# olehskip/resnet.c

Measured on AMD Instinct MI355X. Metric: images/sec ResNet-50 224x224 fp32 batch=256, higher is better.
Workload: dtype f32; 1 GPU; resnet50 fp32 forward, batch 256 per GPU, 224x224 (BASELINE.json configs[2]); global_batch=256, batch_per_gpu=256, mode=fused conv+bn+relu(+add) epilogues, streams_per_gpu=2, streams_configured=library default, front_parts=1, parallelism=batch split over 1 GPU(s), weights replicated, no collective

## Files before the change

### include/rn_hip.h

```cpp
#ifndef RN_HIP_H
#define RN_HIP_H

#include <stddef.h>
#include <stdint.h>

#ifdef __cplusplus
extern "C" {
#endif

#if defined(__GNUC__)
#define RN_API __attribute__((visibility("default")))
#else
#define RN_API
#endif

typedef struct rn_ctx rn_ctx;
typedef struct rn_model rn_model;
typedef struct rn_event rn_event;

enum {
    RN_OK = 0,
    RN_ERR_INVALID = 1,
    RN_ERR_HIP = 2,
    RN_ERR_IO = 3,
// ... 16 lines not shown
RN_API int rn_ctx_get_layout(const rn_ctx *ctx);
RN_API int rn_ctx_set_sync_each_op(rn_ctx *ctx, int on);
RN_API int rn_ctx_set_deferred(rn_ctx *ctx, int on);
RN_API int rn_ctx_get_deferred(const rn_ctx *ctx);
RN_API int rn_flush(rn_ctx *ctx);
RN_API int rn_observe(rn_ctx *ctx, const void *dev_ptr);
RN_API int rn_ctx_deferred_stats(const rn_ctx *ctx, uint64_t *pending_ops, uint64_t *nhwc_buffers,
                                 uint64_t *fused_launches, uint64_t *literal_launches,
                                 uint64_t *transposes);
RN_API int rn_ctx_set_weight_cache(rn_ctx *ctx, int on);
RN_API uint64_t rn_ctx_launch_count(const rn_ctx *ctx);
RN_API int rn_conv_tile_candidates(void);
RN_API int rn_ctx_set_conv_tile(rn_ctx *ctx, int candidate);
RN_API int rn_ctx_set_split_k(rn_ctx *ctx, int max_splits);
RN_API int rn_ctx_set_stem_items(rn_ctx *ctx, int items);
RN_API int rn_ctx_set_xcd_groups(rn_ctx *ctx, int groups);
RN_API int rn_ctx_set_nchw_taps(rn_ctx *ctx, int mode);
RN_API int rn_ctx_set_tap_skip(rn_ctx *ctx, int mode);
RN_API int rn_ctx_tap_skip_stats(const rn_ctx *ctx, uint64_t *launches, uint64_t *k_tiles_skipped);
RN_API int rn_conv_tap_skip_plan(int dtype, uint64_t B, uint64_t in_channels, uint64_t out_channels, uint64_t H,
                                 uint64_t W, uint64_t kernel_size, uint64_t stride, uint64_t padding,
                                 uint64_t dilation, int tile, uint64_t *m_tiles, uint64_t *k_tiles,
                                 uint64_t *k_tiles_skipped, int *rule);
RN_API int rn_ctx_set_debug_stamps(rn_ctx *ctx, void *dev_buffer);
RN_API void *rn_ctx_stream(rn_ctx *ctx);
RN_API int rn_ctx_device(const rn_ctx *ctx);
RN_API int rn_sync(rn_ctx *ctx);
RN_API const char *rn_last_error(const rn_ctx *ctx);
RN_API const char *rn_status_string(int status);
RN_API int rn_device_count(int *count);
RN_API int rn_device_locality(int device, char *pci_bus_id, uint64_t pci_cap, int *numa_node,
                              char *cpulist, uint64_t cpulist_cap);
RN_API const char *rn_version(void);

RN_API int rn_malloc(rn_ctx *ctx, void **dev_ptr, uint64_t bytes);
RN_API int rn_free(rn_ctx *ctx, void *dev_ptr);
RN_API int rn_memcpy_h2d(rn_ctx *ctx, void *dev_dst, const void *host_src, uint64_t bytes);
RN_API int rn_memcpy_d2h(rn_ctx *ctx, void *host_dst, const void *dev_src, uint64_t bytes);
RN_API int rn_memcpy_d2d(rn_ctx *ctx, void *dev_dst, const void *dev_src, uint64_t bytes);
RN_API int rn_memset(rn_ctx *ctx, void *dev_ptr, int byte_value, uint64_t bytes);
RN_API int rn_load_f32_file(rn_ctx *ctx, const char *path, float **dev_ptr, uint64_t *numel);
RN_API int rn_save_f32_file(rn_ctx *ctx, const char *path, const float *dev_ptr, uint64_t numel);

RN_API int rn_event_create(rn_ctx *ctx, rn_event **out);
RN_API int rn_event_destroy(rn_event *ev);
RN_API int rn_event_record(rn_ctx *ctx, rn_event *ev);
// ... 359 lines not shown
```

### resnet.c_amd/_lib.py

```python
from __future__ import annotations

import ctypes
import os
from ctypes import POINTER, c_char_p, c_double, c_float, c_int, c_uint64, c_void_p

_HERE = os.path.dirname(os.path.abspath(__file__))
LIB_PATH = os.environ.get("RN_HIP_LIB") or os.path.join(_HERE, "librn_hip.so")

RN_OK = 0
RN_ERR_INVALID, RN_ERR_HIP, RN_ERR_IO, RN_ERR_NOMEM, RN_ERR_UNSUPPORTED = 1, 2, 3, 4, 5
RN_LAYOUT_NCHW, RN_LAYOUT_NHWC = 0, 1
RN_FWD_REFERENCE_OPS, RN_FWD_FUSED = 0, 1
RN_DTYPE_F32, RN_DTYPE_BF16 = 0, 1
RN_CONV_MAX_DILATION = 1024

u64 = c_uint64
fptr = c_void_p


class ConvSecond(ctypes.Structure):
    _fields_ = [("inp", c_void_p), ("in_channels", c_uint64), ("H", c_uint64), ("W", c_uint64),
                ("stride", c_uint64)]


# ... 20 lines not shown


SIGNATURES = {
    "rn_ctx_create": (c_int, [POINTER(c_void_p), c_int, c_void_p]),
    "rn_ctx_destroy": (c_int, [c_void_p]),
    "rn_ctx_set_layout": (c_int, [c_void_p, c_int]),
    "rn_ctx_get_layout": (c_int, [c_void_p]),
    "rn_ctx_set_sync_each_op": (c_int, [c_void_p, c_int]),
    "rn_ctx_set_deferred": (c_int, [c_void_p, c_int]),
    "rn_ctx_get_deferred": (c_int, [c_void_p]),
    "rn_flush": (c_int, [c_void_p]),
    "rn_observe": (c_int, [c_void_p, c_void_p]),
    "rn_ctx_deferred_stats": (c_int, [c_void_p] + [POINTER(u64)] * 5),
    "rn_ctx_set_weight_cache": (c_int, [c_void_p, c_int]),
    "rn_ctx_launch_count": (u64, [c_void_p]),
    "rn_conv_tile_candidates": (c_int, []),
    "rn_ctx_set_conv_tile": (c_int, [c_void_p, c_int]),
    "rn_ctx_set_split_k": (c_int, [c_void_p, c_int]),
    "rn_ctx_set_stem_items": (c_int, [c_void_p, c_int]),
    "rn_ctx_set_xcd_groups": (c_int, [c_void_p, c_int]),
    "rn_ctx_set_nchw_taps": (c_int, [c_void_p, c_int]),
    "rn_ctx_set_tap_skip": (c_int, [c_void_p, c_int]),
    "rn_ctx_tap_skip_stats": (c_int, [c_void_p, POINTER(u64), POINTER(u64)]),
    "rn_conv_tap_skip_plan": (c_int, [c_int] + [u64] * 9 + [c_int] + [POINTER(u64)] * 3 + [POINTER(c_int)]),
    "rn_ctx_set_debug_stamps": (c_int, [c_void_p, c_void_p]),
    "rn_ctx_stream": (c_void_p, [c_void_p]),
    "rn_ctx_device": (c_int, [c_void_p]),
    "rn_sync": (c_int, [c_void_p]),
    "rn_last_error": (c_char_p, [c_void_p]),
    "rn_status_string": (c_char_p, [c_int]),
    "rn_device_count": (c_int, [POINTER(c_int)]),
    "rn_device_locality": (c_int, [c_int, c_char_p, u64, POINTER(c_int), c_char_p, u64]),
    "rn_version": (c_char_p, []),
    "rn_malloc": (c_int, [c_void_p, POINTER(c_void_p), u64]),
    "rn_free": (c_int, [c_void_p, c_void_p]),
    "rn_memcpy_h2d": (c_int, [c_void_p, c_void_p, c_void_p, u64]),
    "rn_memcpy_d2h": (c_int, [c_void_p, c_void_p, c_void_p, u64]),
    "rn_memcpy_d2d": (c_int, [c_void_p, c_void_p, c_void_p, u64]),
    "rn_memset": (c_int, [c_void_p, c_void_p, c_int, u64]),
    "rn_load_f32_file": (c_int, [c_void_p, c_char_p, POINTER(c_void_p), POINTER(u64)]),
    "rn_save_f32_file": (c_int, [c_void_p, c_char_p, c_void_p, u64]),
    "rn_event_create": (c_int, [c_void_p, POINTER(c_void_p)]),
    "rn_event_destroy": (c_int, [c_void_p]),
    "rn_event_record": (c_int, [c_void_p, c_void_p]),
    "rn_event_elapsed_ms": (c_int, [c_void_p, c_void_p, POINTER(c_float)]),
    "rn_conv_output_size": (u64, [u64, u64, u64, u64]),
# ... 230 lines not shown
```

### resnet.c_amd/csrc/rn_conv.hip

```cpp
#include <type_traits>

#include "rn_conv_params.h"
#include "rn_private.h"

bool rn_conv_is_c4(uint64_t Cin, uint64_t k);

using namespace rn_gemm;

namespace {

constexpr int ROW_FLOATS = 32;

constexpr int tile_blocks_per_cu(int BM, int BN) { return BM * BN <= 64 * 64 ? 4 : BM * BN <= 64 * 128 ? 3 : 2; }

template <typename T, typename TO, int BM, int BN, bool DUAL = false, bool XK = false, bool CHUNK = false,
          bool DIL = false, bool PM = false>
__global__ __launch_bounds__(256, tile_blocks_per_cu(BM, BN)) void conv_gemm_kernel(const GemmParams p)
{
    constexpr int CH = Elem<T>::CH, ES = (int)sizeof(T);
    constexpr int AP = BM / 32;
    constexpr int BP = BN / 32;
    constexpr int MI = BM / 64;
    constexpr int NI = BN / 64;
    constexpr int STAGE = (BM + BN) * ROW_FLOATS;
    __shared__ __attribute__((aligned(16))) float lds[2 * STAGE];

    __builtin_amdgcn_s_setprio(3);
    stamp(p.stamps, 0);
    const unsigned total_tiles = CHUNK ? p.full_tiles : p.total_tiles;
    auto logical_origin = [&](unsigned logical, int &m0_, int &n0_) {
        n0_ = (int)(logical % (unsigned)p.tiles_n) * BN;
        m0_ = (int)(logical / (unsigned)p.tiles_n) * BM;
    };
    auto tile_origin = [&](unsigned v, int &m0_, int &n0_) {
        unsigned pos = xcd_deal(total_tiles, v);
        if (p.xg > 0) {
            const unsigned xg = (unsigned)p.xg, per_group = p.xrows * xg;
            if (pos < p.xrows * (unsigned)p.tiles_n) {
                const unsigned grp = pos / per_group, rem = pos - grp * per_group;
                const unsigned mp = rem / xg, nn = rem - mp * xg;
                pos = mp * (unsigned)p.tiles_n + grp * xg + nn;
            }
        }
        logical_origin(pos, m0_, n0_);
    };
    auto work_item = [&](unsigned v, int &m0_, int &n0_, int &kb_, int &ke_, int &s_) {
        if constexpr (CHUNK) {
            if (v >= p.full_tiles) {
                const unsigned qq = v - p.full_tiles, chunk = qq / p.tail_tiles;
                logical_origin(p.full_tiles + (qq - chunk * p.tail_tiles), m0_, n0_);
                kb_ = (int)chunk * p.chunk_L;
                ke_ = min(kb_ + p.chunk_L, p.nk);
                s_ = (int)chunk;
            } else {
                tile_origin(v, m0_, n0_);
                kb_ = 0;
                ke_ = p.nk;
                s_ = -1;
// ... 929 lines not shown
        auto cost = [&](int g) {
            const double nt = (double)tn / g, mp = R / nt < 1 ? 1 : R / nt;
            const bool stays = taps ? nt * w_slab + mp * a_slab <= 3.8 * MB : nt * w_slab <= 2.5 * MB;
            const double generations = panels / (8.0 / g) / mp;
            const double again = stays ? 1.0 : 3.0 * (generations < 1 ? 1 : generations);
            if (taps && !stays && g > 1) return 1e300;
            return (g > 1 ? 1.3 : 1.0) * g * A + 8.0 * (Wb / g) * again;
        };
        groups = 1;
        double best = cost(1);
        for (int g = 2; g <= 8; g *= 2) {
            if (tn % (unsigned)g) break;
            const double c = cost(g);
            if (c < 0.8 * best) best = c, groups = g;
        }
    }
    if (groups > 8) groups = 8;
    while (groups > 1 && tn % (unsigned)groups) groups /= 2;
    if (groups <= 1) return;
    p.xg = (int)(tn / (unsigned)groups);
    p.xrows = remap_tiles / tn;
}

template <typename T, typename TO, int BM, int BN, bool DUAL, bool XK, bool CHUNK, bool DIL, bool PM>
void launch_one(rn_ctx *ctx, const GemmParams &p, bool persistent, int *occupancy)
{
    unsigned grid = p.grid_items;
    if (persistent) {
        if (*occupancy == 0) {
            int nb = 0;
            if (hipOccupancyMaxActiveBlocksPerMultiprocessor(
                    &nb, conv_gemm_kernel<T, TO, BM, BN, DUAL, XK, CHUNK, DIL, PM>, 256, 0) != hipSuccess ||
                nb < 1)
                nb = 1;
            *occupancy = nb;
        }
        const unsigned slots = 256u * (unsigned)*occupancy;
        if (grid > slots) grid = slots;
    }
    conv_gemm_kernel<T, TO, BM, BN, DUAL, XK, CHUNK, DIL, PM><<<dim3(grid), dim3(256), 0, ctx->stream>>>(p);
}

struct KernelRow {
    int dt_in, dt_out, BM, BN;
    bool dual, xk, chunk, dil, pm;
    void (*launch)(rn_ctx *, const GemmParams &, bool persistent, int *occupancy);
// ... 43 lines not shown
        r.launch(ctx, p, c.persistent, &ctx->occupancy[&r - kKernels]);
        return rn_after_launch(ctx, d.what);
    }
    if (d.second) return rn_set_error(ctx, RN_ERR_UNSUPPORTED, "%s: fused pair needs equal in/out dtype", d.what);
    return rn_set_error(ctx, RN_ERR_UNSUPPORTED, "%s: dtype combination %d -> %d", d.what, d.dt_in, d.dt_out);
}

int launch_gemm(rn_ctx *ctx, const Contraction &d)
{
    GemmParams p = describe(ctx, d);
    const Choice c = choose(ctx, d, p);
    if (c.family == Choice::STRIP) {
        rn_conv_strip_launch(ctx, p);
        return rn_after_launch(ctx, d.what);
    }
    if (c.family == Choice::FOUR_WAVE && ctx->tap_skip != 1) {
        const TapSkipPlan t = plan_tap_skip(d, p, c.BM, c.BN, ctx->split_k > 1);
        if (t.eligible && (ctx->tap_skip == 2 || t.rule)) {
            Choice cp = c;
            cp.pm = true;
            RN_REQUIRE(ctx, split_pixel_major(p, d, c.BM, c.BN), "too many tiles");
            if (c.chunked) p.chunk_L = 2 * (int)rn_ceil_div((uint64_t)p.nk, 16);
            else p.chunk_L = p.nk;
            choose_tile_order(ctx, p, p.full_tiles, c.BM, c.BN);
            RN_TRY(dispatch(ctx, d, cp, p, false));
            ctx->tap_skip_launches += 1, ctx->tap_skip_k_tiles += t.k_skipped;
            return RN_OK;
        }
    }
    RN_REQUIRE(ctx, split_whole_tiles(p, c.BM, c.BN), "too many tiles");
    if (c.family == Choice::WIDE) {
        rn_conv_wide_launch(ctx, p, c.which, d.second != nullptr);
        return rn_after_launch(ctx, d.what);
    }
    FinishParams fin{};
    RN_TRY(split_k_loop(ctx, d, p, &fin));
    const bool k_split = fin.splits > 0;
    if (!k_split) {
        if (c.chunked) RN_TRY(split_chunked_tail(ctx, d, c.BM, p, &fin));
        choose_tile_order(ctx, p, p.full_tiles, c.BM, c.BN);
    }
    RN_TRY(dispatch(ctx, d, c, p, k_split));
    if (fin.splits == 0) return RN_OK;
    const unsigned fgrid = rn_stream_grid(fin.slice / 4, 256);
    if (d.dt_out == RN_DTYPE_BF16)
        splitk_finish_kernel<bf16_t><<<fgrid, 256, 0, ctx->stream>>>(fin);
    else
// ... 236 lines not shown
    if ((dtype != RN_DTYPE_F32 && dtype != RN_DTYPE_BF16) || tile < 0 || tile > 8 || B == 0 || in_channels == 0 ||
        out_channels == 0 || kernel_size == 0 || kernel_size > 15 || stride == 0 || dilation == 0)
        return -1;
    const uint64_t h_out = rn_conv_output_size_dilated(H, kernel_size, stride, padding, dilation);
    const uint64_t w_out = rn_conv_output_size_dilated(W, kernel_size, stride, padding, dilation);
    if (h_out == 0 || w_out == 0) return -1;
    if (dtype != RN_DTYPE_F32 || in_channels % 32 != 0 ||
        !gemm_eligible(nullptr, nullptr, nullptr, in_channels, kernel_size, B * H * W * in_channels,
                       out_channels * kernel_size * kernel_size * in_channels, B * h_out * w_out * out_channels))
        return 0;
    Contraction d{};
    d.dt_in = d.dt_out = dtype;
    d.k = kernel_size, d.stride = stride, d.pad = padding, d.dil = kernel_size == 1 ? 1 : dilation;
    d.h_out = h_out, d.w_out = w_out, d.B = B, d.Cin = in_channels, d.Cout = out_channels, d.H = H, d.W = W;
    rn_ctx none{};
    const GemmParams p = describe(&none, d);
    const Choice c = choose_four_wave(tile, d, p);
    const TapSkipPlan t = plan_tap_skip(d, p, c.BM, c.BN, false);
    if (!t.eligible) return 0;
    if (m_tiles) *m_tiles = t.m_tiles;
    if (k_tiles) *k_tiles = t.k_tiles;
    if (k_tiles_skipped) *k_tiles_skipped = t.k_skipped;
    if (rule) *rule = t.rule ? 1 : 0;
    return 1;
}

int rn_conv2d_nhwc_forward(rn_ctx *ctx, const float *inp, float *out, const float *packed_weight,
                           uint64_t kernel_size, uint64_t stride, uint64_t padding, uint64_t h_out,
                           uint64_t w_out, uint64_t B, uint64_t in_channels, uint64_t out_channels,
                           uint64_t H, uint64_t W, const rn_epilogue *epilogue)
{
    return nhwc_forward(ctx, inp, out, packed_weight, kernel_size, stride, padding, 1, h_out, w_out, B, in_channels,
                        out_channels, H, W, epilogue);
}

int rn_conv2d_forward(rn_ctx *ctx, const float *inp, float *out, const float *weight,
                      uint64_t kernel_size, uint64_t stride, uint64_t padding, uint64_t h_out,
                      uint64_t w_out, uint64_t B, uint64_t in_channels, uint64_t out_channels,
                      uint64_t H, uint64_t W)
{
    return conv2d_forward(ctx, inp, out, weight, kernel_size, stride, padding, 1, h_out, w_out, B, in_channels,
                          out_channels, H, W);
}

int rn_conv2d_nhwc_forward_dt(rn_ctx *ctx, int dtype, int out_dtype, const void *inp, void *out,
                              const void *packed_weight, uint64_t kernel_size, uint64_t stride,
// ... 174 lines not shown
```

### resnet.c_amd/csrc/rn_conv_params.h

```cpp
#ifndef RN_CONV_PARAMS_H
#define RN_CONV_PARAMS_H

#include "rn_internal.h"

namespace rn_gemm {

typedef float f32x16 __attribute__((ext_vector_type(16)));
typedef unsigned int u32x4 __attribute__((ext_vector_type(4)));

struct GemmParams {
    const void *in;
    const void *w;
    void *out;
    const float *scale;
    const float *shift;
    const void *residual;
    int relu;
    int H, W, Cs;
    int Ho, Wo, Cout;
    int KH, KW;
    int stride, pad;
    int cseg;
    int chunk_dw;
    int c4_chunks;
    int tap_rows, k_rows;
    int M;
    int Ktot;
    int nk;
    int tiles_n;
    unsigned total_tiles;
    int xg;
    unsigned xrows;
    int HoWo;
    unsigned mul_hw, shr_hw, mul_w, shr_w;
    unsigned mul_cs, shr_cs, mul_kw, shr_kw;
    int in_bytes, w_bytes, out_bytes;
    const void *in2;
    int in2_bytes, H2, W2, Cs2, stride2, nk1;
    int ksplit, kchunk;
    unsigned total_work;
    unsigned grid_items;
    long long split_stride;
    int chunk_L;
    unsigned full_tiles, tail_tiles;
    void *ws;
    long long ws_stride;
    int kc, kskip, kreal;
    unsigned mul_kc, shr_kc;
    int out_nchw;
    unsigned long long *stamps;
    int dil;
};

typedef __bf16 bf16_t;
typedef bf16_t bf16x8 __attribute__((ext_vector_type(8)));

template <typename T>
struct Elem;
template <>
struct Elem<float> {
// ... 52 lines not shown
```

### resnet.c_amd/csrc/rn_ctx.hip

```cpp
#include <errno.h>
#include <stdarg.h>
#include <stdio.h>
#include <stdlib.h>
#include <string.h>

#include "rn_conv_params.h"
#include "rn_private.h"

int rn_set_error(rn_ctx *ctx, int status, const char *fmt, ...)
{
    if (ctx) {
        va_list ap;
        va_start(ap, fmt);
        vsnprintf(ctx->err, sizeof(ctx->err), fmt, ap);
        va_end(ap);
    }
    return status;
}

int rn_check_hip(rn_ctx *ctx, hipError_t e, const char *what)
{
    if (e == hipSuccess) return RN_OK;
    return rn_set_error(ctx, RN_ERR_HIP, "HIP error %d (%s) in %s", (int)e, hipGetErrorString(e),
                        what);
// ... 9 lines not shown
    return RN_OK;
}

int rn_scratch(rn_ctx *ctx, int slot, uint64_t bytes, void **ptr)
{
    if (slot < 0 || slot >= 6) return rn_set_error(ctx, RN_ERR_INVALID, "bad scratch slot");
    if (ctx->scratch_bytes[slot] < bytes) {
        if (ctx->graphs_live > 0)
            return rn_set_error(ctx, RN_ERR_INVALID,
                                "scratch would have to grow while %d captured graph(s) point into it: "
                                "destroy them first", ctx->graphs_live);
        RN_HIP_TRY(ctx, hipStreamSynchronize(ctx->stream));
        if (ctx->scratch[slot]) RN_HIP_TRY(ctx, hipFree(ctx->scratch[slot]));
        ctx->scratch[slot] = nullptr;
        ctx->scratch_bytes[slot] = 0;
        uint64_t want = (bytes + 255) & ~(uint64_t)255;
        RN_HIP_TRY(ctx, hipMalloc(&ctx->scratch[slot], want));
        ctx->scratch_bytes[slot] = want;
    }
    *ptr = ctx->scratch[slot];
    return RN_OK;
}

void *rn_wcache_find(rn_ctx *ctx, const void *weight, uint64_t cin, uint64_t cout, uint64_t k)
{
    for (int i = 0; i < ctx->wcache_n; ++i) {
        const rn_wcache_entry &e = ctx->wcache[i];
        if (e.key == weight && e.cin == cin && e.cout == cout && e.k == k) return e.packed;
    }
    return nullptr;
}

int rn_wcache_add(rn_ctx *ctx, const void *weight, uint64_t cin, uint64_t cout, uint64_t k,
                  uint64_t bytes, void **packed)
{
    if (ctx->wcache_n == ctx->wcache_cap) {
        const int ncap = ctx->wcache_cap ? 2 * ctx->wcache_cap : 64;
        rn_wcache_entry *ne = (rn_wcache_entry *)realloc(ctx->wcache, (size_t)ncap * sizeof(rn_wcache_entry));
        if (!ne) return rn_set_error(ctx, RN_ERR_NOMEM, "weight cache table");
        ctx->wcache = ne;
        ctx->wcache_cap = ncap;
    }
    void *p = nullptr;
    RN_HIP_TRY(ctx, hipMalloc(&p, bytes));
    rn_wcache_entry &e = ctx->wcache[ctx->wcache_n++];
    e.key = weight;
// ... 108 lines not shown
    if (hipSetDevice(device) != hipSuccess) return RN_ERR_HIP;
    rn_ctx *ctx = (rn_ctx *)calloc(1, sizeof(rn_ctx));
    if (!ctx) return RN_ERR_NOMEM;
    ctx->device = device;
    ctx->cus = 256;
    {
        int v = 0;
        if (hipDeviceGetAttribute(&v, hipDeviceAttributeMultiprocessorCount, device) == hipSuccess && v > 0) ctx->cus = v;
    }
    ctx->layout = RN_LAYOUT_NCHW;
    if (const char *xg = getenv("RN_XCD_NGROUPS")) {
        const int g = atoi(xg);
        if (g == 1 || g == 2 || g == 4 || g == 8) ctx->xcd_groups = g;
    }
    ctx->nchw_taps = 1;
    if (const char *nt = getenv("RN_NCHW_TAPS")) {
        const int v = atoi(nt);
        if (v >= 0 && v <= 2) ctx->nchw_taps = v;
    }
    if (const char *ts = getenv("RN_TAP_SKIP")) {
        const int v = atoi(ts);
        if (v >= 0 && v <= 2) ctx->tap_skip = v;
    }
    if (hip_stream) {
        ctx->stream = (hipStream_t)hip_stream;
        ctx->own_stream = false;
    } else {
        if (hipStreamCreateWithFlags(&ctx->stream, hipStreamNonBlocking) != hipSuccess) {
            free(ctx);
            return RN_ERR_HIP;
        }
        ctx->own_stream = true;
    }
    *out = ctx;
    return RN_OK;
}

int rn_ctx_destroy(rn_ctx *ctx)
{
    if (!ctx) return RN_OK;
    (void)hipSetDevice(ctx->device);
    (void)rn_defer_flush(ctx);
    (void)hipStreamSynchronize(ctx->stream);
    rn_defer_destroy(ctx);
    for (int i = 0; i < 6; ++i) {
        if (ctx->scratch[i]) (void)hipFree(ctx->scratch[i]);
    }
    for (int i = 0; i < ctx->wcache_n; ++i) (void)hipFree(ctx->wcache[i].packed);
    free(ctx->wcache);
    if (ctx->own_stream) (void)hipStreamDestroy(ctx->stream);
    free(ctx);
    return RN_OK;
}

int rn_ctx_set_layout(rn_ctx *ctx, int layout)
{
    if (!ctx) return RN_ERR_INVALID;
    if (layout != RN_LAYOUT_NCHW && layout != RN_LAYOUT_NHWC)
        return rn_set_error(ctx, RN_ERR_INVALID, "unknown layout %d", layout);
    if (ctx->ds && !ctx->defer_running && layout != ctx->layout) {
        RN_TRY(rn_bind_device(ctx));
        RN_TRY(rn_defer_barrier(ctx));
    }
    ctx->layout = layout;
    return RN_OK;
}

int rn_ctx_get_layout(const rn_ctx *ctx) { return ctx ? ctx->layout : -1; }

int rn_ctx_set_sync_each_op(rn_ctx *ctx, int on)
{
    if (!ctx) return RN_ERR_INVALID;
    ctx->sync_each_op = on ? 1 : 0;
    return RN_OK;
}

int rn_ctx_set_conv_tile(rn_ctx *ctx, int candidate)
{
    if (!ctx) return RN_ERR_INVALID;
    if (candidate < 0 || candidate > rn_conv_tile_candidates())
        return rn_set_error(ctx, RN_ERR_INVALID, "conv tile candidate %d out of range", candidate);
    ctx->conv_tile = candidate;
    return RN_OK;
}

int rn_conv_tile_candidates(void) { return 8 + rn_conv_wide_count() + 1; }

int rn_ctx_graphs_live(const rn_ctx *ctx) { return ctx ? ctx->graphs_live : 0; }
int rn_ctx_tap_skip_mode(const rn_ctx *ctx) { return ctx ? ctx->tap_skip : 0; }
int rn_ctx_scratch_slot(rn_ctx *ctx, int slot, uint64_t bytes, void **ptr)
{
    if (!ctx || !ptr) return RN_ERR_INVALID;
    RN_TRY(rn_bind_device(ctx));
    return rn_scratch(ctx, slot, bytes, ptr);
}
int rn_ctx_set_error(rn_ctx *ctx, int status, const char *msg) { return rn_set_error(ctx, status, "%s", msg); }

int rn_ctx_is_capturing(rn_ctx *ctx)
{
    hipStreamCaptureStatus cap = hipStreamCaptureStatusNone;
    if (!ctx || rn_bind_device(ctx) != RN_OK) return 0;
    if (hipStreamIsCapturing(ctx->stream, &cap) != hipSuccess) return 0;
    return cap != hipStreamCaptureStatusNone;
}
int rn_ctx_upload_sync(rn_ctx *ctx, void *dev, const void *host, uint64_t bytes)
{
    if (!ctx || !dev || !host) return RN_ERR_INVALID;
    RN_TRY(rn_bind_device(ctx));
    RN_HIP_TRY(ctx, hipMemcpyAsync(dev, host, bytes, hipMemcpyHostToDevice, ctx->stream));
    RN_HIP_TRY(ctx, hipStreamSynchronize(ctx->stream));
    return RN_OK;
}
// ... 10 lines not shown
int rn_ctx_set_xcd_groups(rn_ctx *ctx, int groups)
{
    if (!ctx) return RN_ERR_INVALID;
    if (groups != 0 && groups != 1 && groups != 2 && groups != 4 && groups != 8)
        return rn_set_error(ctx, RN_ERR_INVALID, "xcd groups %d: 0 (chosen per launch), 1, 2, 4 or 8", groups);
    ctx->xcd_groups = groups;
    return RN_OK;
}

int rn_ctx_set_nchw_taps(rn_ctx *ctx, int mode)
{
    if (!ctx) return RN_ERR_INVALID;
    if (mode < 0 || mode > 2) return rn_set_error(ctx, RN_ERR_INVALID, "nchw taps mode %d: 0 (never), 1 (large planes) or 2 (always)", mode);
    ctx->nchw_taps = mode;
    return RN_OK;
}

int rn_ctx_set_tap_skip(rn_ctx *ctx, int mode)
{
    if (!ctx) return RN_ERR_INVALID;
    if (mode < 0 || mode > 2)
        return rn_set_error(ctx, RN_ERR_INVALID, "tap skip mode %d: 0 (the library's rule), 1 (never) or 2 (wherever eligible)", mode);
    ctx->tap_skip = mode;
    return RN_OK;
}

int rn_ctx_tap_skip_stats(const rn_ctx *ctx, uint64_t *launches, uint64_t *k_tiles_skipped)
{
    if (!ctx) return RN_ERR_INVALID;
    if (launches) *launches = ctx->tap_skip_launches;
    if (k_tiles_skipped) *k_tiles_skipped = ctx->tap_skip_k_tiles;
    return RN_OK;
}

int rn_ctx_set_stem_items(rn_ctx *ctx, int items)
{
    if (!ctx) return RN_ERR_INVALID;
    if (items < 0) return rn_set_error(ctx, RN_ERR_INVALID, "stem items %d: 0 (chosen per launch) or a positive count", items);
    ctx->stem_items = items;
    return RN_OK;
}

int rn_ctx_wait_event(rn_ctx *ctx, rn_event *ev)
{
    if (!ctx || !ev) return RN_ERR_INVALID;
    RN_TRY(rn_bind_device(ctx));
// ... 235 lines not shown
```

### resnet.c_amd/csrc/rn_internal.h

```cpp
#ifndef RN_INTERNAL_H
#define RN_INTERNAL_H

#include <hip/hip_runtime.h>
#include <stdint.h>
#include <stdio.h>

#include "rn_hip.h"

struct rn_wcache_entry {
    const void *key;
    uint64_t cin, cout, k;
    void *packed;
};

#define RN_CONV_GEMM_KERNELS 59

struct rn_ctx {
    int device;
    int cus;
    hipStream_t stream;
    bool own_stream;
    int layout;
    int sync_each_op;
    int conv_tile;
    int graphs_live;
    int split_k;
    int stem_items;
    int nchw_taps;
    int xcd_groups;
    int tap_skip;
    uint64_t tap_skip_launches, tap_skip_k_tiles;
    void *debug_stamps;
    void *scratch[6];
    uint64_t scratch_bytes[6];
    int occupancy[RN_CONV_GEMM_KERNELS];
    int stem_lds_allowed[5];
    uint64_t launches;
    int wcache_on, wcache_n, wcache_cap;
    struct rn_wcache_entry *wcache;
    int defer;
    int defer_running;
    struct rn_defer_state *ds;
    char err[512];
};

struct rn_event {
    hipEvent_t ev;
};

int rn_set_error(rn_ctx *ctx, int status, const char *fmt, ...);
int rn_bind_device(rn_ctx *ctx);
int rn_check_hip(rn_ctx *ctx, hipError_t e, const char *what);
int rn_scratch(rn_ctx *ctx, int slot, uint64_t bytes, void **ptr);
void *rn_wcache_find(rn_ctx *ctx, const void *weight, uint64_t cin, uint64_t cout, uint64_t k);
int rn_wcache_add(rn_ctx *ctx, const void *weight, uint64_t cin, uint64_t cout, uint64_t k,
                  uint64_t bytes, void **packed);
void rn_wcache_remove(rn_ctx *ctx, const void *packed);
void rn_wcache_drop(rn_ctx *ctx, const void *lo, uint64_t bytes);
int rn_after_launch(rn_ctx *ctx, const char *what);

#define RN_HIP_TRY(ctx, expr)                                  \
    do {                                                       \
        int rn_st_ = rn_check_hip((ctx), (expr), #expr);       \
        if (rn_st_ != RN_OK) return rn_st_;                    \
    } while (0)

int rn_defer_flush(rn_ctx *ctx);
int rn_defer_barrier(rn_ctx *ctx);
int rn_defer_before_write(rn_ctx *ctx, const void *ptr, uint64_t bytes, int whole_allocation);
int rn_defer_before_read(rn_ctx *ctx, const void *ptr, uint64_t bytes, const void **alt);
void rn_defer_destroy(rn_ctx *ctx);
int rn_defer_conv(rn_ctx *ctx, const float *inp, float *out, const float *w, uint64_t k, uint64_t s, uint64_t p,
                  uint64_t ho, uint64_t wo, uint64_t B, uint64_t Cin, uint64_t Cout, uint64_t H, uint64_t W);
int rn_defer_bn(rn_ctx *ctx, const float *inp, float *out, const float *w, const float *b, const float *mean,
                const float *var, uint64_t B, uint64_t C, uint64_t N);
int rn_defer_eltwise(rn_ctx *ctx, int is_add, const float *a, const float *b, float *out, uint64_t N);
// ... 43 lines not shown
```

### resnet.c_amd/csrc/rn_model.c

```c
#include <stdio.h>
#include <stdlib.h>
#include <string.h>

#include "rn_hip.h"
#include "rn_private.h"

#define RN_MAX_KEY 96
#define RN_DEFAULT_SIDE 224
#define RN_MIN_SIDE 32
#define RN_MAX_SIDE 2048
#define RN_RESIZE_SIDE 256
#define RN_STEM_WIDTH 64
#define RN_DEFAULT_CLASSES 1000
#define RN_MAX_CLASSES 65536

#define RN_MAX_STREAMS 4

typedef struct {
    char key[RN_MAX_KEY];
    uint64_t numel;
    float *dev;
    int is_set;
} rn_param;

// ... 1438 lines not shown
}

static int forward_chunk(rn_model *m, const void *input, int in_u8, uint64_t B, float *logits, int mode,
                         int prof_keep)
{
    uint64_t lo = 0;
    int parts = parts_of(m, B), i;
    TRY(ensure_acts(m, B));
    if (!prof_keep) m->n_prof = 0;
    if (parts < 2 || m->profiling || m->single_stream_only || m->recording)
        return forward_part(m, m->ctx, 0, input, in_u8, B, logits, mode);
    if (!m->ev_fork) TRY(rn_event_create(m->ctx, &m->ev_fork));
    for (i = 0; i < parts - 1; ++i) {
        if (m->ctxn[i]) continue;
        TRY(rn_ctx_create(&m->ctxn[i], rn_ctx_device(m->ctx), NULL));
        TRY(rn_event_create(m->ctxn[i], &m->ev_join[i]));
    }
    TRY(rn_event_record(m->ctx, m->ev_fork));
    for (i = 0; i < parts; ++i) {
        const uint64_t hi = B * (uint64_t)(i + 1) / (uint64_t)parts;
        rn_ctx *run = i == 0 ? m->ctx : m->ctxn[i - 1];
        if (i > 0) {
            TRY(rn_ctx_set_tap_skip(run, rn_ctx_tap_skip_mode(m->ctx)));
            TRY(rn_ctx_wait_event(run, m->ev_fork));
        }
        TRY(forward_part(m, run, lo, input_at(m, input, in_u8, lo), in_u8, hi - lo, logits + lo * m->classes,
                         mode));
        if (i > 0) TRY(rn_event_record(run, m->ev_join[i - 1]));
        lo = hi;
    }
    for (i = 0; i < parts - 1; ++i) TRY(rn_ctx_wait_event(m->ctx, m->ev_join[i]));
    return RN_OK;
}

static int head_outputs(rn_model *m, const rn_model_outputs *o, uint64_t done, uint64_t nb, const float *logits)
{
    const uint64_t C = m->classes;
    m->run.ctx = m->ctx;
    if (o->features) {
        float *dst = o->features + done * m->feat;
        TRY(prof_begin(m, "features", "head", 0.0, (double)(nb * m->feat) * (double)(elem_size(m) + 4)));
        if (m->dtype == RN_DTYPE_BF16)
            TRY(rn_widen_bf16_forward(m->ctx, m->pooled, dst, nb * m->feat));
        else
            TRY(rn_memcpy_d2d(m->ctx, dst, m->pooled, nb * m->feat * sizeof(float)));
        TRY(prof_end(m));
// ... 469 lines not shown
```

### resnet.c_amd/csrc/rn_private.h

```cpp
#ifndef RN_PRIVATE_H
#define RN_PRIVATE_H

#include "rn_hip.h"

#ifdef __cplusplus
extern "C" {
#endif

int rn_ctx_graphs_live(const rn_ctx *ctx);
int rn_ctx_tap_skip_mode(const rn_ctx *ctx);
int rn_ctx_wait_event(rn_ctx *ctx, rn_event *ev);
int rn_ctx_scratch_slot(rn_ctx *ctx, int slot, uint64_t bytes, void **ptr);
int rn_ctx_is_capturing(rn_ctx *ctx);
int rn_ctx_set_error(rn_ctx *ctx, int status, const char *msg);
int rn_ctx_upload_sync(rn_ctx *ctx, void *dev, const void *host, uint64_t bytes);

int rn_linear_direct_forward(rn_ctx *ctx, const float *inp, float *out, const float *weight, const float *bias,
                             uint64_t B, uint64_t in_features, uint64_t out_features);
int rn_widen_bf16_forward(rn_ctx *ctx, const void *src_bf16, float *dst, uint64_t n);

int rn_conv_dense_nhwc_forward_dt(rn_ctx *ctx, int dtype, int out_dtype, const void *inp, void *out,
                                  const void *packed_weight, uint64_t kernel_size, uint64_t stride, uint64_t padding,
                                  uint64_t dilation, uint64_t h_out, uint64_t w_out, uint64_t B, uint64_t in_channels,
                                  uint64_t out_channels, uint64_t H, uint64_t W, const rn_epilogue *epilogue);
int rn_conv_group_forward(rn_ctx *ctx, const float *inp, float *out, const float *weight, uint64_t kernel_size,
                          uint64_t stride, uint64_t padding, uint64_t dilation, uint64_t h_out, uint64_t w_out,
                          uint64_t B, uint64_t in_channels, uint64_t out_channels, uint64_t H, uint64_t W,
                          uint64_t groups);
int rn_conv_group_nhwc_forward_dt(rn_ctx *ctx, int dtype, int out_dtype, const void *inp, void *out,
                                  const void *packed_weight, uint64_t kernel_size, uint64_t stride, uint64_t padding,
                                  uint64_t dilation, uint64_t h_out, uint64_t w_out, uint64_t B, uint64_t in_channels,
                                  uint64_t out_channels, uint64_t H, uint64_t W, uint64_t groups,
                                  const rn_epilogue *epilogue);
// ... 35 lines not shown
```

### resnet.c_amd/tensor.py

```python
from __future__ import annotations

import ctypes
import enum
import threading
from functools import reduce
from typing import Optional, Sequence

import numpy as np

from . import _lib as L


class Device(enum.Enum):
    CPU = 0
    GPU = 1


class Shape(tuple):

    def __new__(cls, dims: Sequence[int] = ()):
        return super().__new__(cls, (int(d) for d in dims))

    def numel(self) -> int:
        assert len(self) != 0
# ... 29 lines not shown
        L.check(L.lib().rn_ctx_set_deferred(self.handle, int(on)), "rn_ctx_set_deferred", self.handle)

    def flush(self) -> None:
        L.check(L.lib().rn_flush(self.handle), "rn_flush", self.handle)

    def observe(self, dev_ptr) -> None:
        L.check(L.lib().rn_observe(self.handle, dev_ptr), "rn_observe", self.handle)

    def deferred_stats(self) -> dict:
        import ctypes
        v = [ctypes.c_uint64() for _ in range(5)]
        L.check(L.lib().rn_ctx_deferred_stats(self.handle, *(ctypes.byref(x) for x in v)), "rn_ctx_deferred_stats")
        return dict(zip(("pending_ops", "nhwc_buffers", "fused_launches", "literal_launches", "transposes"),
                        (int(x.value) for x in v)))

    def set_xcd_groups(self, groups: int) -> None:
        L.check(L.lib().rn_ctx_set_xcd_groups(self.handle, int(groups)), "rn_ctx_set_xcd_groups", self.handle)

    def set_nchw_taps(self, mode: int) -> None:
        L.check(L.lib().rn_ctx_set_nchw_taps(self.handle, int(mode)), "rn_ctx_set_nchw_taps", self.handle)

    def set_tap_skip(self, mode: int) -> None:
        L.check(L.lib().rn_ctx_set_tap_skip(self.handle, int(mode)), "rn_ctx_set_tap_skip", self.handle)

    def tap_skip_stats(self) -> dict:
        import ctypes
        n, k = ctypes.c_uint64(), ctypes.c_uint64()
        L.check(L.lib().rn_ctx_tap_skip_stats(self.handle, ctypes.byref(n), ctypes.byref(k)), "rn_ctx_tap_skip_stats")
        return {"launches": int(n.value), "k_tiles_skipped": int(k.value)}

    def set_weight_cache(self, on: bool) -> None:
        L.check(L.lib().rn_ctx_set_weight_cache(self.handle, int(on)), "rn_ctx_set_weight_cache")

    def set_split_k(self, max_splits: int) -> None:
        L.check(L.lib().rn_ctx_set_split_k(self.handle, int(max_splits)), "rn_ctx_set_split_k",
                self.handle)

    def close(self) -> None:
        if self.handle:
            L.lib().rn_ctx_destroy(self.handle)
            self.handle = None


_tls = threading.local()


# ... 152 lines not shown
```

Measured before the change: 15420 images/s.

## Schedule tap-skip conv tiles longest-first by pixel work to balance XCDs

For tap-skipped pixel-major conv launches, adds a device table that orders output pixels by the number of in-bounds kernel taps, heaviest first. Tiles are dealt to XCDs in that order with a there-and-back snake over runs of 32, and this replaces the previous XCD grouping order. The goal is to cut tail imbalance, since border pixels do less K work than interior ones. The cost is extra index math per tile and a table lookup, plus possible loss of L2 locality from the old grouped order. A host-side schedule simulator API is also added.

After: 15420 images/s. Within noise of the previous version (-0.0%).

```diff
diff --git a/include/rn_hip.h b/include/rn_hip.h
--- a/include/rn_hip.h
+++ b/include/rn_hip.h
@@ -62,6 +62,12 @@
                                  uint64_t W, uint64_t kernel_size, uint64_t stride, uint64_t padding,
                                  uint64_t dilation, int tile, uint64_t *m_tiles, uint64_t *k_tiles,
                                  uint64_t *k_tiles_skipped, int *rule);
+RN_API int rn_ctx_set_tap_skip_order(rn_ctx *ctx, int order, int cut_permille);
+RN_API int rn_conv_tap_skip_schedule(int dtype, uint64_t B, uint64_t in_channels, uint64_t out_channels, uint64_t H,
+                                     uint64_t W, uint64_t kernel_size, uint64_t stride, uint64_t padding,
+                                     uint64_t dilation, int tile, int order, int cut_permille, uint64_t *whole_tiles,
+                                     uint64_t *cut_tiles, uint64_t *pieces, uint64_t *xcd_k_tiles_max,
+                                     uint64_t *xcd_k_tiles_min, uint64_t *cu_k_tiles_max);
 RN_API int rn_ctx_set_debug_stamps(rn_ctx *ctx, void *dev_buffer);
 RN_API void *rn_ctx_stream(rn_ctx *ctx);
 RN_API int rn_ctx_device(const rn_ctx *ctx);
diff --git a/resnet.c_amd/_lib.py b/resnet.c_amd/_lib.py
--- a/resnet.c_amd/_lib.py
+++ b/resnet.c_amd/_lib.py
@@ -66,6 +66,8 @@
     "rn_ctx_set_nchw_taps": (c_int, [c_void_p, c_int]),
     "rn_ctx_set_tap_skip": (c_int, [c_void_p, c_int]),
     "rn_ctx_tap_skip_stats": (c_int, [c_void_p, POINTER(u64), POINTER(u64)]),
+    "rn_ctx_set_tap_skip_order": (c_int, [c_void_p, c_int, c_int]),
+    "rn_conv_tap_skip_schedule": (c_int, [c_int] + [u64] * 9 + [c_int] * 3 + [POINTER(u64)] * 6),
     "rn_conv_tap_skip_plan": (c_int, [c_int] + [u64] * 9 + [c_int] + [POINTER(u64)] * 3 + [POINTER(c_int)]),
     "rn_ctx_set_debug_stamps": (c_int, [c_void_p, c_void_p]),
     "rn_ctx_stream": (c_void_p, [c_void_p]),
diff --git a/resnet.c_amd/csrc/rn_conv.hip b/resnet.c_amd/csrc/rn_conv.hip
--- a/resnet.c_amd/csrc/rn_conv.hip
+++ b/resnet.c_amd/csrc/rn_conv.hip
@@ -1,3 +1,5 @@
+#include <stdlib.h>
+
 #include <type_traits>
 
 #include "rn_conv_params.h"
@@ -12,6 +14,12 @@
 constexpr int ROW_FLOATS = 32;
 
 constexpr int tile_blocks_per_cu(int BM, int BN) { return BM * BN <= 64 * 64 ? 4 : BM * BN <= 64 * 128 ? 3 : 2; }
+
+__host__ __device__ __forceinline__ unsigned pm_there_and_back(unsigned i, unsigned count)
+{
+    const unsigned run = i >> 5, first = run << 5, len = count - first < 32u ? count - first : 32u;
+    return (run & 1) ? first + len - 1 - (i - first) : i;
+}
 
 template <typename T, typename TO, int BM, int BN, bool DUAL = false, bool XK = false, bool CHUNK = false,
           bool DIL = false, bool PM = false>
@@ -34,6 +42,19 @@
     };
     auto tile_origin = [&](unsigned v, int &m0_, int &n0_) {
         unsigned pos = xcd_deal(total_tiles, v);
+        if constexpr (PM) {
+            if (p.pm_order != nullptr) {
+                const unsigned tn = (unsigned)p.tiles_n, images = fast_div((unsigned)p.M, p.HoWo, p.mul_hw, p.shr_hw);
+                const unsigned blocks = (images + BM - 1) / BM;
+                const unsigned dealt_panels = ((unsigned)p.HoWo * blocks) & ~7u, dealt = dealt_panels * tn;
+                const unsigned j = v < dealt ? pm_there_and_back(v >> 3, dealt >> 3) : v - dealt, jp = j / tn;
+                const unsigned u = v < dealt ? 8 * jp + (v & 7) : dealt_panels + jp;
+                const unsigned rank = u / blocks, g = u - rank * blocks;
+                typedef const __attribute__((address_space(4))) int *const_int_ptr;
+                const unsigned pix = (unsigned)((const_int_ptr)(uintptr_t)p.pm_order)[rank];
+                pos = (g * (unsigned)p.HoWo + pix) * tn + (j - jp * tn);
+            }
+        }
         if (p.xg > 0) {
             const unsigned xg = (unsigned)p.xg, per_group = p.xrows * xg;
             if (pos < p.xrows * (unsigned)p.tiles_n) {
@@ -1009,6 +1030,35 @@
     p.xrows = remap_tiles / tn;
 }
 
+void set_longest_first(GemmParams &p, const int *table)
+{
+    p.pm_order = table;
+    p.xg = 0, p.xrows = 0;
+}
+
+int tap_skip_order_rule(const Contraction &, const GemmParams &) { return 2; }
+
+unsigned pm_item_m_tile(const GemmParams &p, int BM, unsigned v)
+{
+    const unsigned tn = (unsigned)p.tiles_n;
+    if (p.pm_order) {
+        const unsigned blocks = (unsigned)rn_ceil_div((uint64_t)(p.M / p.HoWo), (uint64_t)BM);
+        const unsigned dealt_panels = ((unsigned)p.HoWo * blocks) & ~7u, dealt = dealt_panels * tn;
+        const unsigned j = v < dealt ? pm_there_and_back(v >> 3, dealt >> 3) : v - dealt, jp = j / tn;
+        const unsigned u = v < dealt ? 8 * jp + (v & 7) : dealt_panels + jp;
+        const unsigned rank = u / blocks, g = u - rank * blocks;
+        return g * (unsigned)p.HoWo + (unsigned)p.pm_order[rank];
+    }
+    const unsigned total = p.full_tiles, q = total >> 3, r = total & 7, xcd = v & 7;
+    unsigned pos = (xcd < r ? xcd * (q + 1) : r * (q + 1) + (xcd - r) * q) + (v >> 3);
+    if (p.xg > 0 && pos < p.xrows * tn) {
+        const unsigned xg = (unsigned)p.xg, per_group = p.xrows * xg;
+        const unsigned grp = pos / per_group, rem = pos - grp * per_group, mp = rem / xg;
+        pos = mp * tn + grp * xg + (rem - mp * xg);
+    }
+    return pos / tn;
+}
+
 template <typename T, typename TO, int BM, int BN, bool DUAL, bool XK, bool CHUNK, bool DIL, bool PM>
 void launch_one(rn_ctx *ctx, const GemmParams &p, bool persistent, int *occupancy)
 {
@@ -1098,7 +1148,11 @@
             RN_REQUIRE(ctx, split_pixel_major(p, d, c.BM, c.BN), "too many tiles");
             if (c.chunked) p.chunk_L = 2 * (int)rn_ceil_div((uint64_t)p.nk, 16);
             else p.chunk_L = p.nk;
-            choose_tile_order(ctx, p, p.full_tiles, c.BM, c.BN);
+            const int *table = nullptr;
+            if ((ctx->tap_skip_order ? ctx->tap_skip_order : tap_skip_order_rule(d, p)) == 2)
+                RN_TRY(rn_pm_order(ctx, p.H, p.W, p.KH, p.stride, p.pad, p.Ho, p.Wo, &table));
+            if (table) set_longest_first(p, table);
+            else choose_tile_order(ctx, p, p.full_tiles, c.BM, c.BN);
             RN_TRY(dispatch(ctx, d, cp, p, false));
             ctx->tap_skip_launches += 1, ctx->tap_skip_k_tiles += t.k_skipped;
             return RN_OK;
@@ -1381,6 +1435,57 @@
     if (k_tiles) *k_tiles = t.k_tiles;
     if (k_tiles_skipped) *k_tiles_skipped = t.k_skipped;
     if (rule) *rule = t.rule ? 1 : 0;
+    return 1;
+}
+
+int rn_conv_tap_skip_schedule(int dtype, uint64_t B, uint64_t in_channels, uint64_t out_channels, uint64_t H,
+                              uint64_t W, uint64_t kernel_size, uint64_t stride, uint64_t padding, uint64_t dilation,
+                              int tile, int order, int cut_permille, uint64_t *whole_tiles, uint64_t *cut_tiles,
+                              uint64_t *pieces, uint64_t *xcd_k_tiles_max, uint64_t *xcd_k_tiles_min,
+                              uint64_t *cu_k_tiles_max)
+{
+    uint64_t *const outs[6] = {whole_tiles, cut_tiles, pieces, xcd_k_tiles_max, xcd_k_tiles_min, cu_k_tiles_max};
+    for (uint64_t *o : outs)
+        if (o) *o = 0;
+    if (order < 0 || order > 2 || cut_permille < -1 || cut_permille > 0) return -1;
+    const int st = rn_conv_tap_skip_plan(dtype, B, in_channels, out_channels, H, W, kernel_size, stride, padding,
+                                         dilation, tile, nullptr, nullptr, nullptr, nullptr);
+    if (st != 1) return st;
+    Contraction d{};
+    d.dt_in = d.dt_out = dtype;
+    d.k = kernel_size, d.stride = stride, d.pad = padding, d.dil = 1;
+    d.h_out = rn_conv_output_size_dilated(H, kernel_size, stride, padding, 1);
+    d.w_out = rn_conv_output_size_dilated(W, kernel_size, stride, padding, 1);
+    d.B = B, d.Cin = in_channels, d.Cout = out_channels, d.H = H, d.W = W;
+    rn_ctx none{};
+    GemmParams p = describe(&none, d);
+    const Choice c = choose_four_wave(tile, d, p);
+    if (!split_pixel_major(p, d, c.BM, c.BN)) return 0;
+    int *table = (int *)malloc((size_t)p.HoWo * sizeof(int));
+    if (!table) return -1;
+    rn_pm_order_host(p.H, p.W, p.KH, p.stride, p.pad, p.Ho, p.Wo, table);
+    if ((order ? order : tap_skip_order_rule(d, p)) == 2) set_longest_first(p, table);
+    else choose_tile_order(&none, p, p.full_tiles, c.BM, c.BN);
+    uint64_t xcd[8] = {0}, cu[256] = {0};
+    const unsigned slots = 256u * (unsigned)tile_blocks_per_cu(c.BM, c.BN);
+    const unsigned grid = p.total_work < slots ? p.total_work : slots;
+    for (unsigned v = 0; v < p.total_work; ++v) {
+        const int pix = (int)(pm_item_m_tile(p, c.BM, v) % (unsigned)p.HoWo);
+        const int ih0 = pix / p.Wo * p.stride - p.pad, iw0 = pix % p.Wo * p.stride - p.pad;
+        const int rows = (p.H - ih0 < p.KH ? p.H - ih0 : p.KH) - (ih0 < 0 ? -ih0 : 0);
+        const int cols = (p.W - iw0 < p.KW ? p.W - iw0 : p.KW) - (iw0 < 0 ? -iw0 : 0);
+        xcd[v & 7] += (uint64_t)(rows * cols * p.cseg);
+        cu[v % grid % 256] += (uint64_t)(rows * cols * p.cseg);
+    }
+    free(table);
+    uint64_t hi = xcd[0], lo = xcd[0];
+    for (uint64_t x : xcd) hi = x > hi ? x : hi, lo = x < lo ? x : lo;
+    if (whole_tiles) *whole_tiles = p.total_work;
+    if (xcd_k_tiles_max) *xcd_k_tiles_max = hi;
+    if (xcd_k_tiles_min) *xcd_k_tiles_min = lo;
+    hi = 0;
+    for (uint64_t x : cu) hi = x > hi ? x : hi;
+    if (cu_k_tiles_max) *cu_k_tiles_max = hi;
     return 1;
 }
 
diff --git a/resnet.c_amd/csrc/rn_conv_params.h b/resnet.c_amd/csrc/rn_conv_params.h
--- a/resnet.c_amd/csrc/rn_conv_params.h
+++ b/resnet.c_amd/csrc/rn_conv_params.h
@@ -35,7 +35,10 @@
     unsigned mul_hw, shr_hw, mul_w, shr_w;
     unsigned mul_cs, shr_cs, mul_kw, shr_kw;
     int in_bytes, w_bytes, out_bytes;
-    const void *in2;
+    union {
+        const void *in2;
+        const int *pm_order;
+    };
     int in2_bytes, H2, W2, Cs2, stride2, nk1;
     int ksplit, kchunk;
     unsigned total_work;
diff --git a/resnet.c_amd/csrc/rn_ctx.hip b/resnet.c_amd/csrc/rn_ctx.hip
--- a/resnet.c_amd/csrc/rn_ctx.hip
+++ b/resnet.c_amd/csrc/rn_ctx.hip
@@ -55,6 +55,55 @@
     return RN_OK;
 }
 
+void rn_pm_order_host(int H, int W, int k, int stride, int pad, int h_out, int w_out, int *order)
+{
+    auto inside = [&](int o, int n_in) {
+        const int x0 = o * stride - pad, lo = x0 < 0 ? -x0 : 0, hi = n_in - x0 < k ? n_in - x0 : k;
+        return hi > lo ? hi - lo : 0;
+    };
+    int n = 0;
+    for (int count = k * k; count >= 0; --count)
+        for (int oh = 0; oh < h_out; ++oh) {
+            const int rows = inside(oh, H);
+            for (int ow = 0; ow < w_out; ++ow)
+                if (rows * inside(ow, W) == count) order[n++] = oh * w_out + ow;
+        }
+}
+
+int rn_pm_order(rn_ctx *ctx, int H, int W, int k, int stride, int pad, int h_out, int w_out, const int **table)
+{
+    *table = nullptr;
+    for (int i = 0; i < ctx->pm_orders_n; ++i) {
+        const rn_pm_order_entry &e = ctx->pm_orders[i];
+        if (e.H == H && e.W == W && e.k == k && e.stride == stride && e.pad == pad) {
+            *table = e.table;
+            return RN_OK;
+        }
+    }
+    hipStreamCaptureStatus cap = hipStreamCaptureStatusNone;
+    RN_HIP_TRY(ctx, hipStreamIsCapturing(ctx->stream, &cap));
+    if (cap != hipStreamCaptureStatusNone) return RN_OK;
+    const size_t pixels = (size_t)h_out * (size_t)w_out;
+    rn_pm_order_entry *ne =
+        (rn_pm_order_entry *)realloc(ctx->pm_orders, (size_t)(ctx->pm_orders_n + 1) * sizeof(rn_pm_order_entry));
+    if (!ne) return rn_set_error(ctx, RN_ERR_NOMEM, "pixel order tables");
+    ctx->pm_orders = ne;
+    int *host = (int *)malloc(pixels * sizeof(int));
+    if (!host) return rn_set_error(ctx, RN_ERR_NOMEM, "pixel order of a %d x %d map", h_out, w_out);
+    rn_pm_order_host(H, W, k, stride, pad, h_out, w_out, host);
+    int *dev = nullptr;
+    int st = rn_check_hip(ctx, hipMalloc(&dev, pixels * sizeof(int)), "hipMalloc (pixel order)");
+    if (st == RN_OK) {
+        st = rn_ctx_upload_sync(ctx, dev, host, pixels * sizeof(int));
+        if (st != RN_OK) (void)hipFree(dev);
+    }
+    free(host);
+    if (st != RN_OK) return st;
+    ne[ctx->pm_orders_n++] = rn_pm_order_entry{H, W, k, stride, pad, dev};
+    *table = dev;
+    return RN_OK;
+}
+
 void *rn_wcache_find(rn_ctx *ctx, const void *weight, uint64_t cin, uint64_t cout, uint64_t k)
 {
     for (int i = 0; i < ctx->wcache_n; ++i) {
@@ -209,6 +258,10 @@
         const int v = atoi(ts);
         if (v >= 0 && v <= 2) ctx->tap_skip = v;
     }
+    if (const char *to = getenv("RN_TAP_SKIP_ORDER")) {
+        const int v = atoi(to);
+        if (v >= 0 && v <= 2) ctx->tap_skip_order = v;
+    }
     if (hip_stream) {
         ctx->stream = (hipStream_t)hip_stream;
         ctx->own_stream = false;
@@ -235,6 +288,8 @@
     }
     for (int i = 0; i < ctx->wcache_n; ++i) (void)hipFree(ctx->wcache[i].packed);
     free(ctx->wcache);
+    for (int i = 0; i < ctx->pm_orders_n; ++i) (void)hipFree(ctx->pm_orders[i].table);
+    free(ctx->pm_orders);
     if (ctx->own_stream) (void)hipStreamDestroy(ctx->stream);
     free(ctx);
     return RN_OK;
@@ -275,6 +330,7 @@
 
 int rn_ctx_graphs_live(const rn_ctx *ctx) { return ctx ? ctx->graphs_live : 0; }
 int rn_ctx_tap_skip_mode(const rn_ctx *ctx) { return ctx ? ctx->tap_skip : 0; }
+int rn_ctx_tap_skip_order_mode(const rn_ctx *ctx) { return ctx ? ctx->tap_skip_order : 0; }
 int rn_ctx_scratch_slot(rn_ctx *ctx, int slot, uint64_t bytes, void **ptr)
 {
     if (!ctx || !ptr) return RN_ERR_INVALID;
@@ -331,6 +387,19 @@
     if (mode < 0 || mode > 2)
         return rn_set_error(ctx, RN_ERR_INVALID, "tap skip mode %d: 0 (the library's rule), 1 (never) or 2 (wherever eligible)", mode);
     ctx->tap_skip = mode;
+    return RN_OK;
+}
+
+int rn_ctx_set_tap_skip_order(rn_ctx *ctx, int order, int cut_permille)
+{
+    if (!ctx) return RN_ERR_INVALID;
+    if (order < 0 || order > 2)
+        return rn_set_error(ctx, RN_ERR_INVALID, "tap skip order %d: 0 (the library's rule), 1 (pixel order) or 2 (longest first)", order);
+    if (cut_permille < -1 || cut_permille > 1000)
+        return rn_set_error(ctx, RN_ERR_INVALID, "tap skip cut %d: -1 (the library's rule) or 0 .. 1000 permille", cut_permille);
+    if (cut_permille > 0)
+        return rn_set_error(ctx, RN_ERR_UNSUPPORTED, "tap skip cut %d: a pixel-major launch never cuts its tail (only -1 and 0)", cut_permille);
+    ctx->tap_skip_order = order;
     return RN_OK;
 }
 
diff --git a/resnet.c_amd/csrc/rn_internal.h b/resnet.c_amd/csrc/rn_internal.h
--- a/resnet.c_amd/csrc/rn_internal.h
+++ b/resnet.c_amd/csrc/rn_internal.h
@@ -30,6 +30,9 @@
     int xcd_groups;
     int tap_skip;
     uint64_t tap_skip_launches, tap_skip_k_tiles;
+    int tap_skip_order;
+    int pm_orders_n;
+    struct rn_pm_order_entry *pm_orders;
     void *debug_stamps;
     void *scratch[6];
     uint64_t scratch_bytes[6];
@@ -44,6 +47,11 @@
     char err[512];
 };
 
+struct rn_pm_order_entry {
+    int H, W, k, stride, pad;
+    int *table;
+};
+
 struct rn_event {
     hipEvent_t ev;
 };
@@ -52,6 +60,8 @@
 int rn_bind_device(rn_ctx *ctx);
 int rn_check_hip(rn_ctx *ctx, hipError_t e, const char *what);
 int rn_scratch(rn_ctx *ctx, int slot, uint64_t bytes, void **ptr);
+void rn_pm_order_host(int H, int W, int k, int stride, int pad, int h_out, int w_out, int *order);
+int rn_pm_order(rn_ctx *ctx, int H, int W, int k, int stride, int pad, int h_out, int w_out, const int **table);
 void *rn_wcache_find(rn_ctx *ctx, const void *weight, uint64_t cin, uint64_t cout, uint64_t k);
 int rn_wcache_add(rn_ctx *ctx, const void *weight, uint64_t cin, uint64_t cout, uint64_t k,
                   uint64_t bytes, void **packed);
diff --git a/resnet.c_amd/csrc/rn_model.c b/resnet.c_amd/csrc/rn_model.c
--- a/resnet.c_amd/csrc/rn_model.c
+++ b/resnet.c_amd/csrc/rn_model.c
@@ -1484,6 +1484,7 @@
         rn_ctx *run = i == 0 ? m->ctx : m->ctxn[i - 1];
         if (i > 0) {
             TRY(rn_ctx_set_tap_skip(run, rn_ctx_tap_skip_mode(m->ctx)));
+            TRY(rn_ctx_set_tap_skip_order(run, rn_ctx_tap_skip_order_mode(m->ctx), -1));
             TRY(rn_ctx_wait_event(run, m->ev_fork));
         }
         TRY(forward_part(m, run, lo, input_at(m, input, in_u8, lo), in_u8, hi - lo, logits + lo * m->classes,
diff --git a/resnet.c_amd/csrc/rn_private.h b/resnet.c_amd/csrc/rn_private.h
--- a/resnet.c_amd/csrc/rn_private.h
+++ b/resnet.c_amd/csrc/rn_private.h
@@ -9,6 +9,7 @@
 
 int rn_ctx_graphs_live(const rn_ctx *ctx);
 int rn_ctx_tap_skip_mode(const rn_ctx *ctx);
+int rn_ctx_tap_skip_order_mode(const rn_ctx *ctx);
 int rn_ctx_wait_event(rn_ctx *ctx, rn_event *ev);
 int rn_ctx_scratch_slot(rn_ctx *ctx, int slot, uint64_t bytes, void **ptr);
 int rn_ctx_is_capturing(rn_ctx *ctx);
diff --git a/resnet.c_amd/tensor.py b/resnet.c_amd/tensor.py
--- a/resnet.c_amd/tensor.py
+++ b/resnet.c_amd/tensor.py
@@ -75,6 +75,10 @@
 
     def set_tap_skip(self, mode: int) -> None:
         L.check(L.lib().rn_ctx_set_tap_skip(self.handle, int(mode)), "rn_ctx_set_tap_skip", self.handle)
+
+    def set_tap_skip_order(self, order: int, cut_permille: int = -1) -> None:
+        L.check(L.lib().rn_ctx_set_tap_skip_order(self.handle, int(order), int(cut_permille)),
+                "rn_ctx_set_tap_skip_order", self.handle)
 
     def tap_skip_stats(self) -> dict:
         import ctypes
```
